# devbib/veles

Measured on AMD Instinct MI355X. Metric: samples/sec (whole node) AlexNet-ImageNet training at 1/2/4/8 MI355X, higher is better.
Workload: dtype bf16; 1 GPU; model=alexnet, global_batch=3072, per_gpu_batch=3072, parallelism=dp1, image=227x227x3, grad_allreduce=none (one rank: no collectives)

## Files before the change

csrc/kernels/wgrad_halo.hip:

```cpp
#include "conv_geom.h"

#ifndef HVK_HALO_ABL
#define HVK_HALO_ABL 0
#endif
#include "fp8_common.h"

using namespace hvk;

namespace {

typedef __attribute__((address_space(3))) s16x4 lds_s16x4;

struct HaloGeom {
  int N, H, W, C, OH, OW, OC, Cg, OCg, KH, KW, pt, pl;
  int P;
  int OHW;
  int KK;
  int Wp;
  int WR;
  int SEGP;
  int spi;
  FastDiv fOW, fWp;
};

template <int MT>
__device__ __forceinline__ int a_sw(int r) {
  if constexpr (MT == 128) return r & 7;
  else if constexpr (MT == 96) return (r >> 2) & 1;
  else return (r >> 1) & 3;
}

typedef __attribute__((address_space(3))) uint8_t lds_u8;

__device__ __forceinline__ bf16x8 tr_read(lds_u8* sm, uint32_t o0,
                                          uint32_t o1) {
  s16x4 lo = __builtin_amdgcn_ds_read_tr16_b64_v4i16((lds_s16x4*)(sm + o0));
  s16x4 hi = __builtin_amdgcn_ds_read_tr16_b64_v4i16((lds_s16x4*)(sm + o1));
  typedef __attribute__((ext_vector_type(8))) short s16x8;
  s16x8 v = __builtin_shufflevector(lo, hi, 0, 1, 2, 3, 4, 5, 6, 7);
  return __builtin_bit_cast(bf16x8, v);
}

template <int MT, int NP, int KHT, int KW, int NJW, int PB, bool SEG,
          bool LEAN>
__global__ void __launch_bounds__(256, 2)
wgrad_halo_kernel(const uint16_t* __restrict__ x,
                  const uint16_t* __restrict__ dy, float* __restrict__ ws,
                  float* __restrict__ wsb, HaloGeom g, int mtiles,
                  int cchunks, int kgroups, int tiles, int kspan,
                  int bias) {
  constexpr int NJ = KHT * KW * NP;
  static_assert(2 * NJW >= NJ, "two wave columns cover the n-tiles");
  constexpr int MI = MT / 32;
  constexpr int AP = MT * 2;
  constexpr int ABYTES = 64 * AP;
  constexpr int NA = ABYTES / 1024;
  static_assert(NA % 4 == 0, "A pieces divide over the four waves");
  constexpr int NAW = NA / 4;
  constexpr int BBYTES = NP * PB;
  constexpr int NB = (BBYTES + 1023) / 1024;
  constexpr int NBW = (NB + 3) / 4;
  constexpr int STAGE = ABYTES + NB * 1024;
  static_assert(2 * 2 * STAGE <= 160 * 1024, "two workgroups per CU");
  __shared__ __attribute__((aligned(16))) uint8_t smem[2 * STAGE];

  const int wgid = xcd_remap(blockIdx.x, gridDim.x);
  const int tile = wgid % tiles;
  const int split = wgid / tiles;
  int tt = tile;
  const int kg = tt % kgroups; tt /= kgroups;
  const int cc = tt % cchunks; tt /= cchunks;
  const int mt = tt % mtiles;
  const int gi = tt / mtiles;
  const int total = SEG ? g.N * g.spi : g.P;
  const int pbeg = split * kspan;
  const int pend = min(total, pbeg + kspan);
  if (pbeg >= pend) return;
  const int coff_y = gi * g.OCg + mt * MT;
  const int coff_x = gi * g.Cg + cc * 16 * NP;
  const int kh0 = kg * KHT;

  const int t = threadIdx.x, lane = t & 63;
  const int w = __builtin_amdgcn_readfirstlane(t >> 6);
  const int wr = w >> 1, wc = w & 1;
  const int fr = lane & 15, fq = lane >> 4;
  const int trq = fr >> 2, trp = fr & 3;
  const int q = fq * 4 + trq;

  lds_u8* sm = (lds_u8*)smem;
  const __amdgpu_buffer_rsrc_t ra = dma_rsrc(dy);
  const __amdgpu_buffer_rsrc_t rb = dma_rsrc(x);

  uint32_t a_off[NAW];
  int a_row[NAW];
#pragma unroll
  for (int i = 0; i < NAW; ++i) {
    const int ib = (w * NAW + i) * 1024 + 16 * lane;
    const int r = ib / AP;
    const int pc = (ib - r * AP) >> 4;
    const int lb = (pc >> 1) ^ a_sw<MT>(r);
    const int m = lb * 16 + (pc & 1) * 8;
    a_row[i] = r;
    a_off[i] = (uint32_t)(r * g.OC + coff_y + m) * 2u;
  }
  const int WS = SEG ? KHT * g.SEGP : g.WR * g.Wp;
  int b_rs[NBW];
  uint32_t b_col[NBW];
  uint32_t b_ok[NBW];
  int b_j[NBW];
#pragma unroll
  for (int i = 0; i < NBW; ++i) {
    const int pi = w + 4 * i;
    const int ib = pi * 1024 + 16 * lane;
    const int plane = ib / PB;
    const int wb = ib - plane * PB;
    const int slot = wb >> 5;
    const int half = (wb >> 4) & 1;
// ... 66 lines not shown
          const uint32_t sj = (uint32_t)(ow + b_j[i]);
          const uint32_t rr = fdiv(sj, g.fWp);
          const int col = (int)(sj - rr * (uint32_t)g.Wp);
          const int ih = ihb + (int)rr + b_rs[i];
          const int iw = col - g.pl;
          const bool ok = b_ok[i] && col < g.OW + g.KW - 1 &&
                          (unsigned)iw < (unsigned)g.W &&
                          (unsigned)ih < (unsigned)g.H;
          const uint32_t v = ok ? (nrow + (uint32_t)ih) * rowbytes +
                                      (uint32_t)iw * pixbytes + b_col[i]
                                : kBufOOB;
          dma16(rb, st + ABYTES + (w + 4 * i) * 1024, v);
        }
      }
      return;
    }
    const int rc = g.OH - oh + KHT - 1;
    const int ih_a = oh + kh0 - g.pt;
    const int ih_b = kh0 - g.pt - rc;
    const int gr_a = n * g.H + ih_a;
    const int gr_b = (n + 1) * g.H + ih_b;
    const bool n1ok = n + 1 < g.N;
#pragma unroll
    for (int i = 0; i < NBW; ++i) {
      if (w + 4 * i < NB) {
        const int rs = b_rs[i];
        const bool first = rs < rc;
        const int ih = (first ? ih_a : ih_b) + rs;
        const int gr = (first ? gr_a : gr_b) + rs;
        const bool ok = b_ok[i] && (unsigned)ih < (unsigned)g.H &&
                        (first || n1ok);
        const uint32_t v = ok ? (uint32_t)gr * rowbytes + b_col[i] : kBufOOB;
        dma16(rb, st + ABYTES + (w + 4 * i) * 1024, v);
      }
    }
  };
  auto advance = [&](uint32_t& n, uint32_t& pin, uint32_t& oh,
                     uint32_t& ow) {
    pin += 64;
    if (SEG && pin >= (uint32_t)g.OHW) {
      pin = 0; oh = 0; ow = 0; ++n;
      return;
    }
    if (!SEG && pin >= (uint32_t)g.OHW) pin -= g.OHW;
    ow += 64;
    while (ow >= (uint32_t)g.OW) {
      ow -= g.OW;
      if (++oh == (uint32_t)g.OH) { oh = 0; ++n; }
    }
  };

  constexpr int kNoRow = 0x40000000;
  int l_rs[NBW], l_bj[NBW];
  uint32_t l_inv[NBW];
  int l_b[4];
  uint32_t l_k[4];
  const uint32_t wp32 = (uint32_t)g.Wp * 32u;
  if constexpr (LEAN) {
#pragma unroll
    for (int i = 0; i < NBW; ++i) {
      if constexpr (SEG) {
        const uint32_t aj = fdiv((uint32_t)b_j[i], g.fWp);
        const int bj = b_j[i] - (int)aj * g.Wp;
        const int r = b_rs[i] + (int)aj;
        l_bj[i] = bj;
        l_rs[i] = b_ok[i] ? r : kNoRow;
        l_inv[i] = (uint32_t)r * rowbytes + (uint32_t)(bj - g.pl) * pixbytes +
                   b_col[i];
      } else {
        l_bj[i] = 0;
        l_rs[i] = b_ok[i] ? b_rs[i] : kNoRow;
        l_inv[i] = (uint32_t)b_rs[i] * rowbytes + b_col[i];
      }
    }
#pragma unroll
    for (int i = 0; i < 4; ++i) {
      const uint32_t c = (uint32_t)(q + 16 * i);
      const uint32_t a = fdiv(c, g.fOW);
      const uint32_t b = c - a * (uint32_t)g.OW;
      l_b[i] = (int)b;
      l_k[i] = (a * (uint32_t)g.Wp + b) * 32u + (uint32_t)(trp * 8 + ABYTES);
    }
  }
  struct LeanStep {
    uint32_t n, pin, oh, ow, base, pa;
    int plim;
  };
  const uint32_t q64 = fdiv(64u, g.fOW), r64 = 64u - q64 * (uint32_t)g.OW;
  const uint32_t inc64 = q64 * rowbytes + (SEG ? r64 * pixbytes : 0u);
  const uint32_t inc_row = rowbytes - (SEG ? (uint32_t)g.OW * pixbytes : 0u);
  const uint32_t inc_img = (uint32_t)(g.H - g.OH) * rowbytes;
  const uint32_t astep = 64u * (uint32_t)g.OC * 2u;
  const uint32_t b_delta = (uint32_t)(g.H - g.OH - KHT + 1) * rowbytes;
  const int b_lo = max(0, g.pt - kh0);
  const int b_len = max(0, g.H + g.pt - kh0 - b_lo);
  const int nb_live = (NB - w + 3) >> 2;
  auto lean_first = [&]() {
    LeanStep s;
    s.n = n0; s.pin = pin0; s.oh = oh0; s.ow = ow0;
    s.base = (n0 * (uint32_t)g.H + oh0 + (uint32_t)(kh0 - g.pt)) * rowbytes +
             (SEG ? ow0 * pixbytes : 0u);
    const uint32_t p = n0 * (uint32_t)g.OHW + pin0;
    s.pa = p * (uint32_t)g.OC * 2u;
    s.plim = SEG ? g.OHW - (int)pin0 : pend - (int)p;
    return s;
  };
  auto lean_issue = [&](const LeanStep& s, uint8_t* st) {
    if constexpr ((HVK_HALO_ABL & 1) != 0) return;
    if (s.plim >= 64) {
#pragma unroll
      for (int i = 0; i < NAW; ++i)
        dma16(ra, st + (w * NAW + i) * 1024, s.pa + a_off[i]);
    } else {
#pragma unroll
      for (int i = 0; i < NAW; ++i) {
        const uint32_t v = (a_row[i] < s.plim) ? s.pa + a_off[i] : kBufOOB;
        dma16(ra, st + (w * NAW + i) * 1024, v);
      }
    }
    if constexpr (SEG) {
      const int ihb = (int)s.oh + kh0 - g.pt;
      const uint32_t cw = (uint32_t)max(0, min(g.W, g.OW + g.KW - 1 - g.pl));
      const uint32_t wrapb = rowbytes - (uint32_t)g.Wp * pixbytes;
#pragma unroll
      for (int i = 0; i < NBW; ++i) {
        bool live = true;
        if (i == NBW - 1 && NB % 4 != 0) {
          int nb = nb_live;
          asm volatile("" : "+s"(nb));
          live = i < nb;
        }
        if (live) {
          const int t = l_bj[i] + (int)s.ow;
          const bool c = t >= g.Wp;
          const uint32_t iw = (uint32_t)(t - (c ? g.Wp + g.pl : g.pl));
          const uint32_t ih = (uint32_t)(l_rs[i] + ihb + (c ? 1 : 0));
          uint32_t a = l_inv[i] + s.base + (c ? wrapb : 0u);
          asm("" : "+v"(a));
          const bool ok = (iw < cw) & (ih < (uint32_t)g.H);
          const uint32_t v = ok ? a : kBufOOB;
          dma16(rb, st + ABYTES + (w + 4 * i) * 1024, v);
        }
      }
      return;
    }
    const int rc = g.OH - (int)s.oh + KHT - 1;
    const int ih_a = (int)s.oh + kh0 - g.pt;
    const int a_lo = max(0, -ih_a);
    const uint32_t a_len = (uint32_t)max(0, min(rc, g.H - ih_a) - a_lo);
    const int bl = rc + b_lo;
    const uint32_t bn = s.n + 1 < (uint32_t)g.N ? (uint32_t)b_len : 0u;
    const uint32_t base_b = s.base + b_delta;
#pragma unroll
    for (int i = 0; i < NBW; ++i) {
      bool live = true;
      if (i == NBW - 1 && NB % 4 != 0) {
        int nb = nb_live;
        asm volatile("" : "+s"(nb));
        live = i < nb;
      }
      if (live) {
        const int rs = l_rs[i];
        uint32_t v = (uint32_t)(rs - bl) < bn ? l_inv[i] + base_b : kBufOOB;
        v = (uint32_t)(rs - a_lo) < a_len ? l_inv[i] + s.base : v;
        dma16(rb, st + ABYTES + (w + 4 * i) * 1024, v);
      }
    }
  };
  auto lean_advance = [&](LeanStep& s) {
    if constexpr (SEG) {
      s.pin += 64;
      if (s.pin >= (uint32_t)g.OHW) {
        s.pa += (uint32_t)s.plim * (uint32_t)g.OC * 2u;
        s.pin = 0; s.oh = 0; s.ow = 0; ++s.n;
        s.base = (s.n * (uint32_t)g.H + (uint32_t)(kh0 - g.pt)) * rowbytes;
        s.plim = g.OHW;
        return;
      }
    } else {
      s.pin += 64;
      if (s.pin >= (uint32_t)g.OHW) s.pin -= g.OHW;
    }
    s.pa += astep;
    s.plim -= 64;
    s.oh += q64;
    s.ow += r64;
    s.base += inc64;
    if (s.ow >= (uint32_t)g.OW) {
      s.ow -= g.OW; ++s.oh; s.base += inc_row;
    }
    if (!SEG && s.oh >= (uint32_t)g.OH) {
      s.oh -= g.OH; ++s.n; s.base += inc_img;
    }
  };

  const int nk = SEG ? pend - pbeg : (pend - pbeg + 63) >> 6;
  LeanStep lc{}, ln{};
  if constexpr (LEAN) {
    lc = lean_first();
    lean_issue(lc, smem);
  } else {
    issue(n0, pin0, oh0, ow0, smem);
  }
  asm volatile("s_waitcnt vmcnt(0)" ::: "memory");
  __builtin_amdgcn_s_barrier();
  asm volatile("" ::: "memory");

  uint32_t nn = n0, pinn = pin0, ohn = oh0, own = ow0;
  if constexpr (LEAN) {
    ln = lc;
    lean_advance(ln);
  } else {
    advance(nn, pinn, ohn, own);
  }

  const bool bwave = bias && kg == 0 && cc == 0 && wc == 0;

  auto main_loop = [&](auto wcc, auto with_bias) {
    constexpr int WC = decltype(wcc)::value;
    constexpr bool WB = decltype(with_bias)::value;
    for (int kt = 0; kt < nk; ++kt) {
      const uint32_t cur = (kt & 1) * STAGE;
      if (kt + 1 < nk) {
        if constexpr (LEAN) lean_issue(ln, smem + ((kt + 1) & 1) * STAGE);
        else issue(nn, pinn, ohn, own, smem + ((kt + 1) & 1) * STAGE);
      }
      uint32_t bb[4][KHT];
      const int kp = SEG ? g.SEGP : g.Wp;
      if constexpr (LEAN) {
        const int thr = g.OW - (int)lc.ow;
        const uint32_t dwp = (uint32_t)(g.Wp - g.OW) * 32u;
        const uint32_t sb = cur + lc.ow * 32u;
        const uint32_t wrap = cur + ABYTES + (uint32_t)(g.OH - (int)lc.oh) * wp32;
#pragma unroll
        for (int i = 0; i < 4; ++i) {
          uint32_t base = l_k[i] + (l_b[i] >= thr ? dwp : 0u);
          if constexpr (SEG) {
            base = q < lc.plim - 16 * i ? base : (uint32_t)(trp * 8 + ABYTES);
            base += cur;
          } else {
            base += sb;
            base += base >= wrap ? (uint32_t)(KHT - 1) * wp32 : 0u;
          }
#pragma unroll
          for (int kh = 0; kh < KHT; ++kh) bb[i][kh] = base + kh * kp * 32;
        }
      } else {
#pragma unroll
      for (int i = 0; i < 4; ++i) {
        const uint32_t ow = ow0 + q + 16 * i;
        const uint32_t gr = fdiv(ow, g.fOW);
        const int owr = (int)(ow - gr * (uint32_t)g.OW);
        int slot;
        if constexpr (SEG) {
          slot = pin0 + q + 16 * i < (uint32_t)g.OHW
                     ? (int)gr * g.Wp + owr - (int)ow0 : 0;
        } else {
          slot = ((int)gr + ((oh0 + gr >= (uint32_t)g.OH) ? KHT - 1 : 0)) *
                     g.Wp + owr;
        }
        const uint32_t base = cur + ABYTES + slot * 32 + trp * 8;
#pragma unroll
        for (int kh = 0; kh < KHT; ++kh) bb[i][kh] = base + kh * kp * 32;
      }
      }
#pragma unroll
      for (int ks = 0; ks < 2; ++ks) {
        bf16x8 a[MI];
#pragma unroll
        for (int i = 0; i < MI; ++i) {
          const uint32_t oa = cur + a_frag[i] + ks * 32 * AP;
          a[i] = tr_read(sm, oa, oa + 16 * AP);
        }
#pragma unroll
        for (int j = 0; j < NJW; ++j) {
          const int jg = WC * NJW + j;
          if (jg < NJ) {
            const int tl = jg / NP, pl_ = jg - (jg / NP) * NP;
            const int khl = tl / KW, kwl = tl - (tl / KW) * KW;
            const uint32_t off = kwl * 32 + pl_ * PB;
            const bf16x8 b = tr_read(sm, bb[2 * ks][khl] + off,
                                     bb[2 * ks + 1][khl] + off);
            if constexpr ((HVK_HALO_ABL & 4) != 0) {
              acc[0][j][0] += (float)b[0] + (float)a[0][0];
            } else {
#pragma unroll
              for (int i = 0; i < MI; ++i)
                acc[i][j] = __builtin_amdgcn_mfma_f32_16x16x32_bf16(
                    b, a[i], acc[i][j], 0, 0, 0);
            }
          }
        }
        if constexpr (WB) {
#pragma unroll
          for (int i = 0; i < MI; ++i)
            accb[i] = __builtin_amdgcn_mfma_f32_16x16x32_bf16(ones, a[i],
                                                              accb[i], 0, 0, 0);
        }
      }
      asm volatile("s_waitcnt vmcnt(0)" ::: "memory");
      __builtin_amdgcn_s_barrier();
      asm volatile("" ::: "memory");
      if constexpr (LEAN) {
        lc = ln;
        lean_advance(ln);
      } else {
        ow0 = own; oh0 = ohn; n0 = nn; pin0 = pinn;
        advance(nn, pinn, ohn, own);
      }
    }
  };
  if (wc == 0) {
    if (bwave) main_loop(std::integral_constant<int, 0>{}, std::true_type{});
    else main_loop(std::integral_constant<int, 0>{}, std::false_type{});
  } else {
    main_loop(std::integral_constant<int, 1>{}, std::false_type{});
  }

  const long long sbase = (long long)split * g.OC;
#pragma unroll
  for (int j = 0; j < NJW; ++j) {
    const int jg = wc * NJW + j;
    if (jg >= NJ || ((HVK_HALO_ABL & 2) && acc[0][j][0] != 1234.5f)) continue;
    const int tl = jg / NP, pl_ = jg - (jg / NP) * NP;
    const int khg = kh0 + tl / KW, kwl = tl - (tl / KW) * KW;
    const int ng = (khg * g.KW + kwl) * g.Cg + cc * 16 * NP + pl_ * 16 + fq * 4;
#pragma unroll
    for (int i = 0; i < MI; ++i) {
      const int mg = coff_y + mrow0 + i * 16 + fr;
      *(float4*)(ws + (sbase + mg) * g.KK + ng) =
          make_float4(acc[i][j][0], acc[i][j][1], acc[i][j][2], acc[i][j][3]);
    }
  }
  if (bwave && fq == 0) {
#pragma unroll
    for (int i = 0; i < MI; ++i)
      wsb[sbase + coff_y + mrow0 + i * 16 + fr] = accb[i][0];
  }
}

template <int R>
__global__ void __launch_bounds__(256)
wgrad_finish_kernel(const float* __restrict__ ws, float* __restrict__ dw,
                    long long n4, int splits, const float* __restrict__ wsb,
                    float* __restrict__ db, int oc, int nmain) {
  constexpr int EPB = 256 / R;
  __shared__ float4 red[256];
  const int r = threadIdx.x % R, el = threadIdx.x / R;
  if ((int)blockIdx.x < nmain) {
    const long long e = (long long)blockIdx.x * EPB + el;
    float4 sacc = make_float4(0.f, 0.f, 0.f, 0.f);
    if (e < n4)
      for (int k = r; k < splits; k += R) {
        const float4 v = ((const float4*)ws)[(long long)k * n4 + e];
        sacc.x += v.x; sacc.y += v.y; sacc.z += v.z; sacc.w += v.w;
      }
    if constexpr (R == 1) {
      if (e < n4) {
        float4 d = ((float4*)dw)[e];
        d.x += sacc.x; d.y += sacc.y; d.z += sacc.z; d.w += sacc.w;
        ((float4*)dw)[e] = d;
      }
      return;
    }
    red[threadIdx.x] = sacc;
    __syncthreads();
    if (r == 0 && e < n4) {
      float4 t = red[el * R];
#pragma unroll
      for (int i = 1; i < R; ++i) {
        const float4 v = red[el * R + i];
        t.x += v.x; t.y += v.y; t.z += v.z; t.w += v.w;
      }
      float4 d = ((float4*)dw)[e];
      d.x += t.x; d.y += t.y; d.z += t.z; d.w += t.w;
      ((float4*)dw)[e] = d;
    }
    return;
  }
  if (db == nullptr) return;
  const int m = ((int)blockIdx.x - nmain) * EPB + el;
  float sb = 0.f;
  if (m < oc)
    for (int k = r; k < splits; k += R) sb += wsb[(long long)k * oc + m];
  float* rf = (float*)red;
  rf[threadIdx.x] = sb;
  __syncthreads();
  if (r == 0 && m < oc) {
    float t = rf[el * R];
    for (int i = 1; i < R; ++i) t += rf[el * R + i];
// ... 276 lines not shown
          accb[i] = __builtin_amdgcn_mfma_scale_f32_16x16x128_f8f6f4(
              ones, a[i], accb[i], FX, FDY, 0, 127, 0, 127);
      }
      asm volatile("s_waitcnt vmcnt(0)" ::: "memory");
      __builtin_amdgcn_s_barrier();
      asm volatile("" ::: "memory");
      ow0 = own; oh0 = ohn; n0 = nn; pin0 = pinn;
      advance(nn, pinn, ohn, own);
    }
  };
  if (wc == 0) {
    if (bwave) main_loop(std::integral_constant<int, 0>{}, std::true_type{});
    else main_loop(std::integral_constant<int, 0>{}, std::false_type{});
  } else {
    main_loop(std::integral_constant<int, 1>{}, std::false_type{});
  }

  const float sdv = fp8_scale(sdys, hist, fmax_dy);
  const float alpha = 1.f / (sdv * fp8_scale(sxs, hist, fmax_x));
  const long long sbase = (long long)split * g.OC;
#pragma unroll
  for (int jn = 0; jn < NJW; ++jn) {
    const int jg = wc * NJW + jn;
    if (jg >= NJ) continue;
    const int tl = jg / NP, pl_ = jg - (jg / NP) * NP;
    const int khg = kh0 + tl / KW, kwl = tl - (tl / KW) * KW;
    const int ng = (khg * g.KW + kwl) * g.Cg + cc * 16 * NP + pl_ * 16 + fg * 4;
#pragma unroll
    for (int i = 0; i < MI; ++i) {
      const int mg = coff_y + mrow0 + i * 16 + fr;
      *(float4*)(ws + (sbase + mg) * g.KK + ng) =
          make_float4(acc[i][jn][0] * alpha, acc[i][jn][1] * alpha,
                      acc[i][jn][2] * alpha, acc[i][jn][3] * alpha);
    }
  }
  if (bwave && fg == 0) {
#pragma unroll
    for (int i = 0; i < MI; ++i)
      wsb[sbase + coff_y + mrow0 + i * 16 + fr] = accb[i][0] / sdv;
  }
}

struct Plan {
  int var;
  int MT, NP, KHT, PB;
  int tiles, mtiles, cchunks, kgroups;
  int splits, kspan;
  HaloGeom g;
};

constexpr int kSlots = 512;
int g_halo_pad = 2;
int g_halo_lean = 1;

Plan make_plan(int N, int H, int W, int C, int OC, int KH, int KW, int pt,
               int pl, int OH, int OW, int groups, int splits,
               bool fp8 = false) {
  const int STEP = fp8 ? 128 : 64, SLOT = fp8 ? 16 : 32, ES = fp8 ? 1 : 2;
  Plan p{};
  const int Cg = C / groups, OCg = OC / groups;
  HaloGeom& g = p.g;
  g.N = N; g.H = H; g.W = W; g.C = C; g.OH = OH; g.OW = OW; g.OC = OC;
  g.Cg = Cg; g.OCg = OCg; g.KH = KH; g.KW = KW; g.pt = pt; g.pl = pl;
  g.P = N * OH * OW;
  g.KK = KH * KW * Cg;
  g.Wp = OW + (fp8 ? 16 : std::max(g_halo_pad, KW - 1));
  g.fOW = make_fastdiv(OW);
  if (OH * OW < STEP || KW > 9 || C % 16 != 0 || OC % 16 != 0) return p;
  if ((long long)N * H * W * C * ES >= kBufMaxBytes ||
      (long long)g.P * OC * ES >= kBufMaxBytes)
    return p;
  g.OHW = OH * OW;
  g.fWp = make_fastdiv(g.Wp);
  const int span = (OW - 1 + STEP - 1) / OW + 1;
  const int cross = (OH * OW) % STEP != 0 ? 2 : 1;
  const int spi = (g.OHW + STEP - 1) / STEP;
  int dmax = 0;
  for (int st = 0; st < spi; ++st) {
    const int pin = STEP * st, last = min(pin + STEP - 1, g.OHW - 1);
    const int d = (last / OW - pin / OW) * g.Wp + last % OW - pin % OW;
    dmax = max(dmax, d);
  }
  struct Cand { int var, MT, NP, KHT, KW, PB, seg; };
  const Cand cands16[] = {
      {1, 128, 2, 3, 3, 7168, 0},
      {5, 128, 2, 3, 3, 7168, 1},
      {4, 128, 2, 3, 3, 10240, 0},
      {2, 96, 2, 3, 3, 7168, 0},
      {7, 96, 3, 3, 3, 8192, 1},
      {6, 64, 4, 3, 3, 7168, 1},
      {3, 128, 3, 1, 5, 5120, 0},
  };
  const Cand cands8[] = {
      {101, 128, 2, 3, 3, 9216, 0},
      {102, 128, 2, 3, 3, 7168, 1},
      {103, 64, 4, 3, 3, 7168, 1},
  };
  const Cand* cands = fp8 ? cands8 : cands16;
  const int ncand = fp8 ? 3 : 7;
  for (int ci = 0; ci < ncand; ++ci) {
    const Cand& c = cands[ci];
    if (KW != c.KW || KH % c.KHT || OCg % c.MT || Cg % (16 * c.NP)) continue;
    if (c.seg) {
      if (spi * STEP * 100 > g.OHW * 103) continue;
      const int segp = dmax + KW;
      if (c.KHT * segp * SLOT > c.PB) continue;
      g.SEGP = segp;
      g.spi = spi;
      g.WR = 0;
    } else {
      const int WR = span + cross * (c.KHT - 1);
      if (WR * g.Wp * SLOT > c.PB) continue;
      g.WR = WR;
      g.SEGP = 0;
      g.spi = 0;
    }
    p.var = c.var; p.MT = c.MT; p.NP = c.NP; p.KHT = c.KHT; p.PB = c.PB;
    break;
  }
  if (!p.var) return p;
  p.mtiles = OCg / p.MT;
  p.cchunks = Cg / (16 * p.NP);
  p.kgroups = KH / p.KHT;
  p.tiles = groups * p.mtiles * p.cchunks * p.kgroups;
  const bool seg = g.SEGP > 0;
  const int steps = seg ? N * spi : (g.P + STEP - 1) / STEP;
  int s = splits > 0 ? splits : kSlots / p.tiles;
  s = max(1, min(s, steps));
  const int ks = (steps + s - 1) / s;
  p.kspan = seg ? ks : ks * STEP;
  p.splits = (steps + ks - 1) / ks;
  return p;
}

}

static long long finish(float* ws, float* wsb, float* dW, float* dbias, int OC,
                 long long kk, int splits, hipStream_t s);

HVK_API long long hvk_conv_wgrad_halo(const void* X, const void* dY, float* dW,
                                      float* dbias, float* ws, int N, int H,
                                      int W, int C, int OC, int KH, int KW,
                                      int pt, int pl, int OH, int OW,
                                      int groups, int splits, hipStream_t s) {
  Plan p = make_plan(N, H, W, C, OC, KH, KW, pt, pl, OH, OW, groups, splits);
  if (!p.var) return -1;
  const long long kk = (long long)KH * KW * (C / groups);
  const long long need = (long long)p.splits * OC * kk + (long long)p.splits * OC;
  if (ws == nullptr) return need;
  if (((uintptr_t)X & 15) || ((uintptr_t)dY & 15)) return -1;
  float* wsb = ws + (long long)p.splits * OC * kk;
  dim3 grid((unsigned)(p.tiles * p.splits)), blk(256);
  const int bias = dbias != nullptr;
  const uint16_t* x = (const uint16_t*)X;
  const uint16_t* dy = (const uint16_t*)dY;
#define HALO_GO1(MT, NP, KHT, KW, NJW, PB, SEG, LEAN)                          \
  hipLaunchKernelGGL(                                                          \
      (wgrad_halo_kernel<MT, NP, KHT, KW, NJW, PB, SEG, LEAN>), grid, blk, 0,  \
      s, x, dy, ws, wsb, p.g, p.mtiles, p.cchunks, p.kgroups, p.tiles,         \
      p.kspan, bias)
#define HALO_GO(MT, NP, KHT, KW, NJW, PB, SEG)                                 \
  if (g_halo_lean) HALO_GO1(MT, NP, KHT, KW, NJW, PB, SEG, true);              \
  else HALO_GO1(MT, NP, KHT, KW, NJW, PB, SEG, false)
  switch (p.var) {
    case 1: HALO_GO(128, 2, 3, 3, 9, 7168, false); break;
    case 2: HALO_GO(96, 2, 3, 3, 9, 7168, false); break;
    case 3: HALO_GO(128, 3, 1, 5, 8, 5120, false); break;
    case 4: HALO_GO(128, 2, 3, 3, 9, 10240, false); break;
    case 5: HALO_GO(128, 2, 3, 3, 9, 7168, true); break;
    case 6: HALO_GO(64, 4, 3, 3, 18, 7168, true); break;
    case 7: HALO_GO(96, 3, 3, 3, 14, 8192, true); break;
    default: return -1;
  }
#undef HALO_GO
#undef HALO_GO1
  hipError_t e = launch_status(s);
  if (e != hipSuccess) return (long long)e;
  return finish(ws, wsb, dW, dbias, OC, kk, p.splits, s);
}

static long long finish(float* ws, float* wsb, float* dW, float* dbias, int OC,
                 long long kk, int splits, hipStream_t s) {
  const long long n4 = (long long)OC * kk / 4;
  const int R = (splits >= 64 && n4 < (1 << 17)) ? 16
              : (splits >= 16 && n4 < (1 << 19)) ? 4 : 1;
  const int epb = 256 / R;
  const int nmain = (int)((n4 + epb - 1) / epb);
  const int nb = dbias ? (OC + epb - 1) / epb : 0;
  auto fk = R == 16 ? wgrad_finish_kernel<16>
          : R == 4 ? wgrad_finish_kernel<4> : wgrad_finish_kernel<1>;
  hipLaunchKernelGGL(fk, dim3(nmain + nb), dim3(256), 0, s, ws, dW, n4,
                     splits, wsb, dbias, OC, nmain);
  return (long long)launch_status(s);
}

HVK_API void hvk_halo_pitch_pad(int p) { g_halo_pad = p; }

HVK_API void hvk_halo_lean(int on) { g_halo_lean = on; }

HVK_API int hvk_conv_wgrad_halo_splits(int N, int H, int W, int C, int OC,
                                       int KH, int KW, int pt, int pl, int OH,
                                       int OW, int groups, int splits) {
  Plan p = make_plan(N, H, W, C, OC, KH, KW, pt, pl, OH, OW, groups, splits);
  return p.var ? p.splits : -1;
}

HVK_API long long hvk_conv_wgrad_halo_fp8(
    const void* X8, const void* dY8, float* dW, float* dbias, float* ws,
    int N, int H, int W, int C, int OC, int KH, int KW, int pt, int pl,
    int OH, int OW, int groups, int splits, int fx, int fdy, const float* sxs,
    const float* sdys, int hist, float fmax_x, float fmax_dy, hipStream_t s) {
  Plan p = make_plan(N, H, W, C, OC, KH, KW, pt, pl, OH, OW, groups, splits,
                     true);
  if (!p.var || (fx != 0 && fx != 1) || (fdy != 0 && fdy != 1)) return -1;
  const long long kk = (long long)KH * KW * (C / groups);
  const long long need = (long long)p.splits * OC * kk + (long long)p.splits * OC;
  if (ws == nullptr) return need;
  if (((uintptr_t)X8 & 15) || ((uintptr_t)dY8 & 15)) return -1;
  float* wsb = ws + (long long)p.splits * OC * kk;
  dim3 grid((unsigned)(p.tiles * p.splits)), blk(256);
  const int bias = dbias != nullptr;
  const uint8_t* x = (const uint8_t*)X8;
  const uint8_t* dy = (const uint8_t*)dY8;
#define HALO8_GO(MT, NP, KHT, KW, NJW, PB, SEG, FX, FDY)                       \
  hipLaunchKernelGGL(                                                          \
      (wgrad_halo8_kernel<MT, NP, KHT, KW, NJW, PB, SEG, FX, FDY>), grid, blk, \
      0, s, x, dy, ws, wsb, p.g, p.mtiles, p.cchunks, p.kgroups, p.tiles,      \
      p.kspan, bias, sxs, sdys, hist, fmax_x, fmax_dy)
#define HALO8_FMT(MT, NP, KHT, KW, NJW, PB, SEG)                               \
  if (fx == 0 && fdy == 1) HALO8_GO(MT, NP, KHT, KW, NJW, PB, SEG, 0, 1);     \
  else if (fx == 0 && fdy == 0) HALO8_GO(MT, NP, KHT, KW, NJW, PB, SEG, 0, 0); \
  else if (fx == 1 && fdy == 1) HALO8_GO(MT, NP, KHT, KW, NJW, PB, SEG, 1, 1); \
  else HALO8_GO(MT, NP, KHT, KW, NJW, PB, SEG, 1, 0)
  switch (p.var) {
    case 101: HALO8_FMT(128, 2, 3, 3, 9, 9216, false); break;
    case 102: HALO8_FMT(128, 2, 3, 3, 9, 7168, true); break;
    case 103: HALO8_FMT(64, 4, 3, 3, 18, 7168, true); break;
    default: return -1;
  }
#undef HALO8_FMT
#undef HALO8_GO
  hipError_t e = launch_status(s);
  if (e != hipSuccess) return (long long)e;
  return finish(ws, wsb, dW, dbias, OC, kk, p.splits, s);
}
```

veles_amd/ops/__init__.py:

```python
from __future__ import annotations

import math
import os
import struct

import torch
import torch.nn.functional as F

from veles_amd.ops import _lib
from veles_amd.ops._lib import available, require_library

__all__ = ["ACT", "gemm", "linear_fwd", "conv_out_size", "conv_fwd",
           "conv_dgrad", "conv_wgrad", "col_sum", "row_sum", "act_fwd",
           "act_bwd", "pool_fwd", "pool_bwd", "lrn_fwd", "lrn_bwd",
           "softmax_ce", "mse", "sgd_update", "dropout", "xorshift1024star",
           "xorshift128plus", "join", "cast", "fill_minibatch",
           "mean_disp_normalize", "act_code", "kohonen_coords",
           "kohonen_argmin", "kohonen_update", "lstm_fwd", "lstm_bwd",
           "rbm_layout", "rbm_uniforms", "rbm_sample", "rbm_grad",
           "bn_partials", "batchnorm_fwd", "batchnorm_bwd", "attention_fwd",
           "attention_bwd", "mha_fwd", "mha_bwd", "attn_head_dim"]

DT = {torch.float32: 0, torch.bfloat16: 1, torch.uint8: 2, torch.int32: 3,
      torch.float16: 4}
# ... 999 lines not shown
        if isinstance(col, (S2DImage, PaddedImage)):
            col = None
        if col is not None:
            K = KH * KW * Cg
            M = N * OH * OW
            sp = splits or wgrad_splits(M, OC, K, 1)
            gemm(dy.reshape(M, OC), col[:, :K], trans_a=True,
                 out=dw.view(OC, K), accumulate=True, splits=sp,
                 bias_grad=dbias)
            return dw
        if needs_im2col(C, groups):
            runp = (KW * C + 7) // 8 * 8
            sp = splits or _wgrad_splits_for(
                x, dy, dw, sliding, padding, groups,
                (N * OH * OW, OC, KH * runp + 1, 1))
            _lib_call("hvk_conv_wgrad_run", _p(x), _p(dy), _p(dw), _p(dbias),
                      N, H, W, C, OC, KH, KW, sy, sx, pt, pl, OH, OW,
                      int(sp), _s(x))
            return dw
        if (sy, sx) == (1, 1) and _halo_wgrad(x, dy, dw, dbias, N, H, W, C,
                                               OC, KH, KW, pt, pl, OH, OW,
                                               groups, splits):
            return dw
        if splits is None:
            splits = _wgrad_splits_for(
                x, dy, dw, sliding, padding, groups,
                (N * OH * OW, OC // groups, KH * KW * Cg + 1, groups))
        _lib_call("hvk_conv_wgrad", _p(x), _p(dy), _p(dw), N, H, W, C, OC, KH,
                  KW, sy, sx, pt, pl, OH, OW, groups, int(splits), _p(dbias),
                  _s(x))
        return dw
    xp = F.pad(_nchw(x), (pl, pr, pt, pb))
    g = torch.nn.grad.conv2d_weight(xp, (OC, Cg, KH, KW), _nchw(dy),
                                    stride=(sy, sx), groups=groups)
    dw += g.permute(0, 2, 3, 1)
    if dbias is not None:
        dbias += dy.float().reshape(-1, OC).sum(0)
    return dw


_HALO_WGRAD = os.environ.get("VELES_AMD_HALO_WGRAD", "1") != "0"


def set_halo_wgrad(on):
    global _HALO_WGRAD
    _HALO_WGRAD = bool(on)


def set_halo_wgrad_lean(on):
    if _lib.available():
        _lib.lib().hvk_halo_lean(int(bool(on)))


def _halo_wgrad(x, dy, dw, dbias, N, H, W, C, OC, KH, KW, pt, pl, OH, OW,
                groups, splits=None):
    if not _HALO_WGRAD or x.dtype != torch.bfloat16 or \
            dy.dtype != torch.bfloat16 or not dw.is_contiguous() or \
            not x.is_contiguous() or not dy.is_contiguous() or \
            x.data_ptr() % 16 or dy.data_ptr() % 16:
        return False
    from veles_amd.ops import _lib
    fn = _lib.lib().hvk_conv_wgrad_halo
    geo = (N, H, W, C, OC, KH, KW, pt, pl, OH, OW, groups,
           int(splits) if splits else 0)
    need = fn(_p(x), _p(dy), _p(dw), _p(dbias), None, *geo, _s(x))
    if need < 0:
        return False
    ws = _grow_ws("wgrad_halo_ws", int(need), torch.float32, x.device)
    rc = fn(_p(x), _p(dy), _p(dw), _p(dbias), _p(ws), *geo, _s(x))
    _lib.check(int(rc), "hvk_conv_wgrad_halo")
    return True


_WGRAD_BLOCKS = int(os.environ.get("HVK_WGRAD_BLOCKS", "512"))


def _wgrad_splits_for(x, dy, dw, sliding, padding, groups, shape):
    from veles_amd.ops import autotune
    default = wgrad_splits(*shape)
    autotune.log_call("wgrad", shape, {
        "x": tuple(x if isinstance(x, tuple) else x.shape), "dy": tuple(dy.shape), "dw": tuple(dw.shape),
        "sliding": tuple(sliding), "padding": tuple(padding),
        "groups": groups, "default": default})
    t = autotune.lookup("wgrad", *shape)
    if deterministic():
        return 1
    return default if t is None else max(1, t)


def wgrad_splits(P, M, N, groups, target_blocks=None):
    if deterministic():
        return 1
    target_blocks = target_blocks or _WGRAD_BLOCKS
    tiles = ((M + 127) // 128) * ((N + 127) // 128) * groups
    splits = max(1, min(target_blocks // max(tiles, 1), P // 256))
    return splits


def col_sum(x2d, out=None, scale=1.0, accumulate=False):
    R, C = x2d.shape
    if out is None:
        out = torch.zeros(C, dtype=torch.float32, device=x2d.device)
    elif not accumulate:
        out.zero_()
    if _gpu(x2d) and not deterministic():
        _lib_call("hvk_col_sum", _p(x2d), DT[x2d.dtype], R, C, _p(out),
# ... 2501 lines not shown
```

veles_amd/ops/_lib.py:

```python
from __future__ import annotations

import ctypes
import os
import threading

from veles_amd.error import KernelLibraryMissing

_HERE = os.path.dirname(os.path.abspath(__file__))
LIB_PATH = os.environ.get("HVK_LIBRARY", os.path.join(_HERE, "libhvk.so"))

_lib = None
_lock = threading.Lock()

P = ctypes.c_void_p
I = ctypes.c_int
L = ctypes.c_longlong
F = ctypes.c_float
D = ctypes.c_double
U = ctypes.c_uint

_SIGS = {
    "hvk_gemm": [I, I, I, I, I, P, I, P, I, P, I, I, I, F, F, P, I, I, P, I, I,
                 I, P, P],
    "hvk_gemm_splitk": [I, I, I, I, I, P, I, P, I, P, I, I, F, P, I, P, I, I,
# ... 39 lines not shown
    "hvk_space_to_depth": [P, P] + [I] * 9 + [P],
    "hvk_s2d_weights": [P, P] + [I] * 5 + [P],
    "hvk_s2d_grad_fold": [P, P] + [I] * 6 + [P],
    "hvk_pool_fwd": [P, P, P] + [I] * 13 + [P],
    "hvk_pool_bwd": [P, P, P] + [I] * 13 + [P, I, P],
    "hvk_lrn_fwd": [P, P, L, I, I, F, F, F, P],
    "hvk_lrn_bwd": [P, P, P, L, I, I, F, F, F, P, I, P],
    "hvk_lrn_pool_fwd": [P, P, P] + [I] * 9 + [F, F, F, P],
    "hvk_lrn_pool_bwd": [P, P, P, P] + [I] * 9 + [F, F, F, P, I, P],
    "hvk_pool2_fwd": [P, P] + [I] * 5 + [P],
    "hvk_pool2_fwd_q8": [P, P] + [I] * 5 + [P, P, P, F, I, I, P],
    "hvk_stochastic_pool": [P, P, P] + [I] * 12 + [P, P],
    "hvk_pool2_bwd": [P, P, P] + [I] * 5 + [P, I, P],
    "hvk_pool2_bwd_q8": [P, P, P] + [I] * 5 + [P, I, P, P, P, F, I, I, P],
    "hvk_lrn_pool_fwd_u8": [P, P, P] + [I] * 7 + [F, F, F, P],
    "hvk_lrn_pool_bwd_u8": [P, P, P, P] + [I] * 7 + [F, F, F, P, I, P],
    "hvk_gemm_f32": [I, I, I, I, I, P, I, P, I, P, I, F, F, I, P],
    "hvk_gemm_f64": [I, I, I, I, I, P, I, P, I, P, I, D, D, I, P],
    "hvk_fp8_quant": [P, I, L, P, I, P, I, F, I, P],
    "hvk_fp8_amax": [P, I, L, P, I, P],
    "hvk_fp8_roll": [P, I, I, I, I, P, P],
    "hvk_fp8_roll_dev": [P, I, I, P, P, P],
    "hvk_gemm_fp8": [I, I, I, P, I, I, P, I, I, P, I, P, I, P, I, I, P, P, I,
                     F, F, P],
    "hvk_conv_fwd_fp8": [P, P, P, P] + [I] * 17 + [P, P, I, F, F,
                                                  P, P, P, F, I, P],
    "hvk_conv_dgrad_fp8": [P, P, P] + [I] * 14 + [P, I, I, I, P, P, I, F, F,
                           P, P, P, F, I, P],
    "hvk_conv_wgrad_fp8": [P, P, P, P] + [I] * 17 + [P, P, I, F, F, P],
    "hvk_conv_wgrad_halo": [P, P, P, P, P] + [I] * 13 + [P],
    "hvk_conv_wgrad_halo_splits": [I] * 13,
    "hvk_conv_wgrad_halo_fp8": [P, P, P, P, P] + [I] * 15 + [P, P, I, F, F,
                                                            P],
    "hvk_conv_fwd_hc": [P, P, P, P] + [I] * 13 + [P, P],
    "hvk_conv_dgrad_hc": [P, P, P] + [I] * 12 + [P, I, P, P],
    "hvk_conv_dgrad_hc_w": [P, P, P] + [I] * 12 + [P, I, P, P],
    "hvk_conv_hc_wpack_bytes": [I] * 14,
    "hvk_hc_variant": [I],
    "hvk_hc_pitch_pad": [I],
    "hvk_hc32": [I],
    "hvk_halo_pitch_pad": [I],
    "hvk_hc32_ts": [I],
    "hvk_transpose_colsum": [P, I, I, P, P, I, P, P],
    "hvk_hc_last_variant": [],
    "hvk_set_pool_bwd_variant": [I],
    "hvk_hc_ablation": [I],
    "hvk_take_last_error": [],
    "hvk_end_stream_capture": [P],
    "hvk_stream_create": [],
}
_OPTIONAL = {
    "hvk_hc32_handover": [I],
    "hvk_halo_lean": [I],
    "hvk_hc_max_wgs": [I],
    "hvk_hc_stamps": [P],
    "hvk_kohonen_argmin": [P, I, P, I, I, I, I, P, P, P, P, I, P],
    "hvk_kohonen_update": [P, I, P, P, P, I, I, I, I, F, F, P, I, P],
    "hvk_lstm_step_fwd": [I, I, I] + [P, L] * 7 + [P],
    "hvk_lstm_step_bwd": [I, I, I] + [P, L] * 9 + [P],
    "hvk_recurrent_fn": [I, P, P, L, P],
    "hvk_gru_step_fwd": [I, I] + [P, L] * 8 + [P, P],
    "hvk_gru_step_bwd": [I, I] + [P, L] * 10 + [P],
    "hvk_lstm_step_fwd2": [I, I, I] + [P, L] * 14 + [P],
    "hvk_lstm_step_bwd2": [I, I, I] + [P, L] * 18 + [P],
    "hvk_gru_step_fwd2": [I, I] + ([P, L] * 8 + [P]) * 2 + [P],
    "hvk_gru_step_bwd2": [I, I] + [P, L] * 20 + [P],
    "hvk_rbm_sample": [I, I, I, I, P, L, P, L, P, P, L, P, L, U, P, L, P],
    "hvk_rbm_grad_splits": [I, I, I, I],
    "hvk_rbm_grad": [I, I, I] + [P, L] * 4 + [P, F, P, I, P],
    "hvk_solver4": [P, P, P, P, P, P, I, L, F, L, P, F, P],
    "hvk_grad_sqnorm": [P, L, P, I, P, P],
    "hvk_bn_partials": [L, I, I],
    "hvk_bn_vec": [P, L, I],
    "hvk_bn_stats": [P, L, L, I, I, P, P, P, P, F, F, P, P, P, P, P],
    "hvk_bn_fold": [P, P, P, P, I, F, P, P],
    "hvk_bn_apply": [P, L, P, L, L, I, P, I, P],
    "hvk_bn_bwd": [P, L] * 5 + [L, I, I, P, P, P, P, P, I, I, I, P, P, P],
    "hvk_attn_tile": [I],
    "hvk_attn_fwd": [P, L] * 4 + [P, I, I, I, I, I, P],
    "hvk_attn_bwd_delta": [P, L] * 2 + [P, I, I, I, I, P],
    "hvk_attn_bwd_dkv": [P, L] * 4 + [P, P] + [P, L] * 2 + [I, I, I, I, I, P],
    "hvk_attn_bwd_dq": [P, L] * 4 + [P, P] + [P, L] + [I, I, I, I, I, P],
}
_PTR_RET = {"hvk_stream_create"}
_LL_RET = {"hvk_conv_wgrad_halo", "hvk_conv_wgrad_halo_fp8",
           "hvk_conv_hc_wpack_bytes"}


def _load():
    global _lib
    with _lock:
        if _lib is not None:
            return _lib
        if not os.path.exists(LIB_PATH):
            return None
        lib = ctypes.CDLL(LIB_PATH)
        for name, sig in _SIGS.items():
            fn = getattr(lib, name, None)
            if fn is None:
                raise KernelLibraryMissing("%s lacks %s - rebuild with python "
                                           "-m veles_amd.ops.build" %
                                           (LIB_PATH, name))
            fn.argtypes = sig
            fn.restype = ctypes.c_void_p if name in _PTR_RET else \
                ctypes.c_longlong if name in _LL_RET else ctypes.c_int
        for name, sig in _OPTIONAL.items():
# ... 52 lines not shown
```

Baseline: 207,600 samples/s.

## Split halo wgrad double buffer into two LDS objects with unrolled even/odd steps

Adds an STG variant of the lean halo weight-gradient kernel. The two pipeline stages become separate LDS arrays and the main loop is unrolled into even/odd steps, so each step uses a constant buffer base instead of computing a per-iteration offset. It also switches to a typed LDS buffer-load DMA, packs row and column indices into one register to cut VGPR use, reads both k-slices of A fragments up front, and uses a precise waitcnt encoding. It is enabled by default for variants 1, 2 and 7. The cost is more code and register pressure from holding both A slices, plus a risk of changing how waits interleave with MFMA work.

```diff
diff --git a/csrc/kernels/wgrad_halo.hip b/csrc/kernels/wgrad_halo.hip
--- a/csrc/kernels/wgrad_halo.hip
+++ b/csrc/kernels/wgrad_halo.hip
@@ -32,6 +32,12 @@
 
 typedef __attribute__((address_space(3))) uint8_t lds_u8;
 
+__device__ __forceinline__ void dma16l(__amdgpu_buffer_rsrc_t r, lds_u8* lds,
+                                       uint32_t voff) {
+  __builtin_amdgcn_raw_ptr_buffer_load_lds(
+      r, (__attribute__((address_space(3))) void*)lds, 16, voff, 0, 0, 0);
+}
+
 __device__ __forceinline__ bf16x8 tr_read(lds_u8* sm, uint32_t o0,
                                           uint32_t o1) {
   s16x4 lo = __builtin_amdgcn_ds_read_tr16_b64_v4i16((lds_s16x4*)(sm + o0));
@@ -42,7 +48,7 @@
 }
 
 template <int MT, int NP, int KHT, int KW, int NJW, int PB, bool SEG,
-          bool LEAN>
+          bool LEAN, bool STG>
 __global__ void __launch_bounds__(256, 2)
 wgrad_halo_kernel(const uint16_t* __restrict__ x,
                   const uint16_t* __restrict__ dy, float* __restrict__ ws,
@@ -62,7 +68,11 @@
   constexpr int NBW = (NB + 3) / 4;
   constexpr int STAGE = ABYTES + NB * 1024;
   static_assert(2 * 2 * STAGE <= 160 * 1024, "two workgroups per CU");
-  __shared__ __attribute__((aligned(16))) uint8_t smem[2 * STAGE];
+  static_assert(LEAN || !STG, "the two-object stages are the lean loop's");
+  static_assert(STAGE % 1024 == 0, "whole DMA pieces per stage");
+  __shared__ __attribute__((aligned(1024))) uint8_t
+      smem[STG ? STAGE : 2 * STAGE];
+  __shared__ __attribute__((aligned(1024))) uint8_t smem1[STG ? STAGE : 16];
 
   const int wgid = xcd_remap(blockIdx.x, gridDim.x);
   const int tile = wgid % tiles;
@@ -235,6 +245,7 @@
 
   constexpr int kNoRow = 0x40000000;
   int l_rs[NBW], l_bj[NBW];
+  uint32_t l_pk[NBW];
   uint32_t l_inv[NBW];
   int l_b[4];
   uint32_t l_k[4];
@@ -248,10 +259,12 @@
         const int r = b_rs[i] + (int)aj;
         l_bj[i] = bj;
         l_rs[i] = b_ok[i] ? r : kNoRow;
+        l_pk[i] = b_ok[i] ? (uint32_t)bj | (uint32_t)r << 16 : 0xffffffffu;
         l_inv[i] = (uint32_t)r * rowbytes + (uint32_t)(bj - g.pl) * pixbytes +
                    b_col[i];
       } else {
         l_bj[i] = 0;
+        l_pk[i] = 0;
         l_rs[i] = b_ok[i] ? b_rs[i] : kNoRow;
         l_inv[i] = (uint32_t)b_rs[i] * rowbytes + b_col[i];
       }
@@ -263,6 +276,10 @@
       const uint32_t b = c - a * (uint32_t)g.OW;
       l_b[i] = (int)b;
       l_k[i] = (a * (uint32_t)g.Wp + b) * 32u + (uint32_t)(trp * 8 + ABYTES);
+      if constexpr (STG) {
+        l_k[i] |= b << 16;
+        asm volatile("" : "+v"(l_k[i]));
+      }
     }
   }
   struct LeanStep {
@@ -288,17 +305,20 @@
     s.plim = SEG ? g.OHW - (int)pin0 : pend - (int)p;
     return s;
   };
-  auto lean_issue = [&](const LeanStep& s, uint8_t* st) {
+  auto lean_issue = [&](const LeanStep& s, lds_u8* st) {
     if constexpr ((HVK_HALO_ABL & 1) != 0) return;
     if (s.plim >= 64) {
 #pragma unroll
       for (int i = 0; i < NAW; ++i)
-        dma16(ra, st + (w * NAW + i) * 1024, s.pa + a_off[i]);
+        dma16l(ra, st + (w * NAW + i) * 1024, s.pa + a_off[i]);
     } else {
+      int la = lane;
+      if constexpr (STG) asm volatile("" : "+v"(la));
 #pragma unroll
       for (int i = 0; i < NAW; ++i) {
-        const uint32_t v = (a_row[i] < s.plim) ? s.pa + a_off[i] : kBufOOB;
-        dma16(ra, st + (w * NAW + i) * 1024, v);
+        const int r = STG ? ((w * NAW + i) * 1024 + 16 * la) / AP : a_row[i];
+        const uint32_t v = (r < s.plim) ? s.pa + a_off[i] : kBufOOB;
+        dma16l(ra, st + (w * NAW + i) * 1024, v);
       }
     }
     if constexpr (SEG) {
@@ -314,15 +334,17 @@
           live = i < nb;
         }
         if (live) {
-          const int t = l_bj[i] + (int)s.ow;
+          const int bj = STG ? (int)(l_pk[i] & 0xffffu) : l_bj[i];
+          const int rs = STG ? (int)(l_pk[i] >> 16) : l_rs[i];
+          const int t = bj + (int)s.ow;
           const bool c = t >= g.Wp;
           const uint32_t iw = (uint32_t)(t - (c ? g.Wp + g.pl : g.pl));
-          const uint32_t ih = (uint32_t)(l_rs[i] + ihb + (c ? 1 : 0));
+          const uint32_t ih = (uint32_t)(rs + ihb + (c ? 1 : 0));
           uint32_t a = l_inv[i] + s.base + (c ? wrapb : 0u);
           asm("" : "+v"(a));
           const bool ok = (iw < cw) & (ih < (uint32_t)g.H);
           const uint32_t v = ok ? a : kBufOOB;
-          dma16(rb, st + ABYTES + (w + 4 * i) * 1024, v);
+          dma16l(rb, st + ABYTES + (w + 4 * i) * 1024, v);
         }
       }
       return;
@@ -346,7 +368,7 @@
         const int rs = l_rs[i];
         uint32_t v = (uint32_t)(rs - bl) < bn ? l_inv[i] + base_b : kBufOOB;
         v = (uint32_t)(rs - a_lo) < a_len ? l_inv[i] + s.base : v;
-        dma16(rb, st + ABYTES + (w + 4 * i) * 1024, v);
+        dma16l(rb, st + ABYTES + (w + 4 * i) * 1024, v);
       }
     }
   };
@@ -377,15 +399,24 @@
     }
   };
 
+  auto stage_wait = [&]() {
+    if constexpr (STG) {
+      asm volatile("" ::: "memory");
+      __builtin_amdgcn_s_waitcnt(0x0f70);
+      asm volatile("" ::: "memory");
+    } else {
+      asm volatile("s_waitcnt vmcnt(0)" ::: "memory");
+    }
+  };
   const int nk = SEG ? pend - pbeg : (pend - pbeg + 63) >> 6;
   LeanStep lc{}, ln{};
   if constexpr (LEAN) {
     lc = lean_first();
-    lean_issue(lc, smem);
+    lean_issue(lc, sm);
   } else {
     issue(n0, pin0, oh0, ow0, smem);
   }
-  asm volatile("s_waitcnt vmcnt(0)" ::: "memory");
+  stage_wait();
   __builtin_amdgcn_s_barrier();
   asm volatile("" ::: "memory");
 
@@ -397,16 +428,28 @@
     advance(nn, pinn, ohn, own);
   }
 
-  const bool bwave = bias && kg == 0 && cc == 0 && wc == 0;
+  constexpr int BWC = STG ? 1 : 0;
+  const bool bwave = bias && kg == 0 && cc == 0 && wc == BWC;
 
   auto main_loop = [&](auto wcc, auto with_bias) {
     constexpr int WC = decltype(wcc)::value;
     constexpr bool WB = decltype(with_bias)::value;
-    for (int kt = 0; kt < nk; ++kt) {
-      const uint32_t cur = (kt & 1) * STAGE;
-      if (kt + 1 < nk) {
-        if constexpr (LEAN) lean_issue(ln, smem + ((kt + 1) & 1) * STAGE);
-        else issue(nn, pinn, ohn, own, smem + ((kt + 1) & 1) * STAGE);
+    auto step = [&](auto par, int kt, bool more) {
+      constexpr int PAR = decltype(par)::value;
+      const uint32_t cur = STG ? 0 : (kt & 1) * STAGE;
+      lds_u8* sc;
+      if constexpr (!STG) sc = sm;
+      else if constexpr (PAR == 0) sc = (lds_u8*)smem;
+      else sc = (lds_u8*)smem1;
+      if (more) {
+        if constexpr (STG) {
+          if constexpr (PAR == 0) lean_issue(ln, (lds_u8*)smem1);
+          else lean_issue(ln, (lds_u8*)smem);
+        } else if constexpr (LEAN) {
+          lean_issue(ln, sm + ((kt + 1) & 1) * STAGE);
+        } else {
+          issue(nn, pinn, ohn, own, smem + ((kt + 1) & 1) * STAGE);
+        }
       }
       uint32_t bb[4][KHT];
       const int kp = SEG ? g.SEGP : g.Wp;
@@ -417,7 +460,12 @@
         const uint32_t wrap = cur + ABYTES + (uint32_t)(g.OH - (int)lc.oh) * wp32;
 #pragma unroll
         for (int i = 0; i < 4; ++i) {
-          uint32_t base = l_k[i] + (l_b[i] >= thr ? dwp : 0u);
+          uint32_t base;
+          if constexpr (STG)
+            base = (l_k[i] & 0xffffu) +
+                   (l_k[i] >= (uint32_t)thr << 16 ? dwp : 0u);
+          else
+            base = l_k[i] + (l_b[i] >= thr ? dwp : 0u);
           if constexpr (SEG) {
             base = q < lc.plim - 16 * i ? base : (uint32_t)(trp * 8 + ABYTES);
             base += cur;
@@ -447,14 +495,15 @@
         for (int kh = 0; kh < KHT; ++kh) bb[i][kh] = base + kh * kp * 32;
       }
       }
-#pragma unroll
-      for (int ks = 0; ks < 2; ++ks) {
-        bf16x8 a[MI];
-#pragma unroll
-        for (int i = 0; i < MI; ++i) {
-          const uint32_t oa = cur + a_frag[i] + ks * 32 * AP;
-          a[i] = tr_read(sm, oa, oa + 16 * AP);
-        }
+      if constexpr (STG) {
+        bf16x8 a[2][MI];
+#pragma unroll
+        for (int ks = 0; ks < 2; ++ks)
+#pragma unroll
+          for (int i = 0; i < MI; ++i) {
+            const uint32_t oa = a_frag[i] + ks * 32 * AP;
+            a[ks][i] = tr_read(sc, oa, oa + 16 * AP);
+          }
 #pragma unroll
         for (int j = 0; j < NJW; ++j) {
           const int jg = WC * NJW + j;
@@ -462,7 +511,46 @@
             const int tl = jg / NP, pl_ = jg - (jg / NP) * NP;
             const int khl = tl / KW, kwl = tl - (tl / KW) * KW;
             const uint32_t off = kwl * 32 + pl_ * PB;
-            const bf16x8 b = tr_read(sm, bb[2 * ks][khl] + off,
+#pragma unroll
+            for (int ks = 0; ks < 2; ++ks) {
+              const bf16x8 b = tr_read(sc, bb[2 * ks][khl] + off,
+                                       bb[2 * ks + 1][khl] + off);
+              if constexpr ((HVK_HALO_ABL & 4) != 0) {
+                acc[0][j][0] += (float)b[0] + (float)a[ks][0][0];
+              } else {
+#pragma unroll
+                for (int i = 0; i < MI; ++i)
+                  acc[i][j] = __builtin_amdgcn_mfma_f32_16x16x32_bf16(
+                      b, a[ks][i], acc[i][j], 0, 0, 0);
+              }
+            }
+          }
+        }
+        if constexpr (WB) {
+#pragma unroll
+          for (int ks = 0; ks < 2; ++ks)
+#pragma unroll
+            for (int i = 0; i < MI; ++i)
+              accb[i] = __builtin_amdgcn_mfma_f32_16x16x32_bf16(
+                  ones, a[ks][i], accb[i], 0, 0, 0);
+        }
+      } else {
+#pragma unroll
+      for (int ks = 0; ks < 2; ++ks) {
+        bf16x8 a[MI];
+#pragma unroll
+        for (int i = 0; i < MI; ++i) {
+          const uint32_t oa = cur + a_frag[i] + ks * 32 * AP;
+          a[i] = tr_read(sc, oa, oa + 16 * AP);
+        }
+#pragma unroll
+        for (int j = 0; j < NJW; ++j) {
+          const int jg = WC * NJW + j;
+          if (jg < NJ) {
+            const int tl = jg / NP, pl_ = jg - (jg / NP) * NP;
+            const int khl = tl / KW, kwl = tl - (tl / KW) * KW;
+            const uint32_t off = kwl * 32 + pl_ * PB;
+            const bf16x8 b = tr_read(sc, bb[2 * ks][khl] + off,
                                      bb[2 * ks + 1][khl] + off);
             if constexpr ((HVK_HALO_ABL & 4) != 0) {
               acc[0][j][0] += (float)b[0] + (float)a[0][0];
@@ -481,25 +569,44 @@
                                                               accb[i], 0, 0, 0);
         }
       }
-      asm volatile("s_waitcnt vmcnt(0)" ::: "memory");
+      }
+      stage_wait();
       __builtin_amdgcn_s_barrier();
       asm volatile("" ::: "memory");
       if constexpr (LEAN) {
         lc = ln;
         lean_advance(ln);
+        if constexpr (STG)
+          asm volatile("" : "+s"(ln.n), "+s"(ln.pin), "+s"(ln.oh), "+s"(ln.ow),
+                            "+s"(ln.base), "+s"(ln.pa), "+s"(ln.plim));
       } else {
         ow0 = own; oh0 = ohn; n0 = nn; pin0 = pinn;
         advance(nn, pinn, ohn, own);
       }
+    };
+    constexpr std::integral_constant<int, 0> even{};
+    constexpr std::integral_constant<int, 1> odd{};
+    if constexpr (STG) {
+      int kt = 0;
+      for (; kt + 1 < nk; kt += 2) {
+        step(even, kt, true);
+        step(odd, kt + 1, kt + 2 < nk);
+      }
+      if (kt < nk) step(even, kt, false);
+    } else {
+      for (int kt = 0; kt < nk; ++kt) step(even, kt, kt + 1 < nk);
     }
   };
-  if (wc == 0) {
-    if (bwave) main_loop(std::integral_constant<int, 0>{}, std::true_type{});
-    else main_loop(std::integral_constant<int, 0>{}, std::false_type{});
+  if (wc == BWC) {
+    if (bwave) main_loop(std::integral_constant<int, BWC>{}, std::true_type{});
+    else main_loop(std::integral_constant<int, BWC>{}, std::false_type{});
   } else {
-    main_loop(std::integral_constant<int, 1>{}, std::false_type{});
-  }
-
+    main_loop(std::integral_constant<int, 1 - BWC>{}, std::false_type{});
+  }
+
+  int te = threadIdx.x;
+  if constexpr (STG) asm volatile("" : "+v"(te));
+  const int fre = STG ? te & 15 : fr, fqe = STG ? (te & 63) >> 4 : fq;
   const long long sbase = (long long)split * g.OC;
 #pragma unroll
   for (int j = 0; j < NJW; ++j) {
@@ -507,18 +614,18 @@
     if (jg >= NJ || ((HVK_HALO_ABL & 2) && acc[0][j][0] != 1234.5f)) continue;
     const int tl = jg / NP, pl_ = jg - (jg / NP) * NP;
     const int khg = kh0 + tl / KW, kwl = tl - (tl / KW) * KW;
-    const int ng = (khg * g.KW + kwl) * g.Cg + cc * 16 * NP + pl_ * 16 + fq * 4;
+    const int ng = (khg * g.KW + kwl) * g.Cg + cc * 16 * NP + pl_ * 16 + fqe * 4;
 #pragma unroll
     for (int i = 0; i < MI; ++i) {
-      const int mg = coff_y + mrow0 + i * 16 + fr;
+      const int mg = coff_y + mrow0 + i * 16 + fre;
       *(float4*)(ws + (sbase + mg) * g.KK + ng) =
           make_float4(acc[i][j][0], acc[i][j][1], acc[i][j][2], acc[i][j][3]);
     }
   }
-  if (bwave && fq == 0) {
+  if (bwave && fqe == 0) {
 #pragma unroll
     for (int i = 0; i < MI; ++i)
-      wsb[sbase + coff_y + mrow0 + i * 16 + fr] = accb[i][0];
+      wsb[sbase + coff_y + mrow0 + i * 16 + fre] = accb[i][0];
   }
 }
 
@@ -901,6 +1008,7 @@
 constexpr int kSlots = 512;
 int g_halo_pad = 2;
 int g_halo_lean = 1;
+int g_halo_stages = 1;
 
 Plan make_plan(int N, int H, int W, int C, int OC, int KH, int KW, int pt,
                int pl, int OH, int OW, int groups, int splits,
@@ -1003,24 +1111,30 @@
   const int bias = dbias != nullptr;
   const uint16_t* x = (const uint16_t*)X;
   const uint16_t* dy = (const uint16_t*)dY;
-#define HALO_GO1(MT, NP, KHT, KW, NJW, PB, SEG, LEAN)                          \
+#define HALO_GO1(MT, NP, KHT, KW, NJW, PB, SEG, LEAN, STG)                     \
   hipLaunchKernelGGL(                                                          \
-      (wgrad_halo_kernel<MT, NP, KHT, KW, NJW, PB, SEG, LEAN>), grid, blk, 0,  \
-      s, x, dy, ws, wsb, p.g, p.mtiles, p.cchunks, p.kgroups, p.tiles,         \
-      p.kspan, bias)
+      (wgrad_halo_kernel<MT, NP, KHT, KW, NJW, PB, SEG, LEAN, STG>), grid,     \
+      blk, 0, s, x, dy, ws, wsb, p.g, p.mtiles, p.cchunks, p.kgroups,          \
+      p.tiles, p.kspan, bias)
 #define HALO_GO(MT, NP, KHT, KW, NJW, PB, SEG)                                 \
-  if (g_halo_lean) HALO_GO1(MT, NP, KHT, KW, NJW, PB, SEG, true);              \
-  else HALO_GO1(MT, NP, KHT, KW, NJW, PB, SEG, false)
+  if (g_halo_lean && g_halo_stages)                                            \
+    HALO_GO1(MT, NP, KHT, KW, NJW, PB, SEG, true, true);                       \
+  else if (g_halo_lean) HALO_GO1(MT, NP, KHT, KW, NJW, PB, SEG, true, false);  \
+  else HALO_GO1(MT, NP, KHT, KW, NJW, PB, SEG, false, false)
+#define HALO_GO_ONE(MT, NP, KHT, KW, NJW, PB, SEG)                             \
+  if (g_halo_lean) HALO_GO1(MT, NP, KHT, KW, NJW, PB, SEG, true, false);       \
+  else HALO_GO1(MT, NP, KHT, KW, NJW, PB, SEG, false, false)
   switch (p.var) {
     case 1: HALO_GO(128, 2, 3, 3, 9, 7168, false); break;
     case 2: HALO_GO(96, 2, 3, 3, 9, 7168, false); break;
-    case 3: HALO_GO(128, 3, 1, 5, 8, 5120, false); break;
-    case 4: HALO_GO(128, 2, 3, 3, 9, 10240, false); break;
-    case 5: HALO_GO(128, 2, 3, 3, 9, 7168, true); break;
-    case 6: HALO_GO(64, 4, 3, 3, 18, 7168, true); break;
+    case 3: HALO_GO_ONE(128, 3, 1, 5, 8, 5120, false); break;
+    case 4: HALO_GO_ONE(128, 2, 3, 3, 9, 10240, false); break;
+    case 5: HALO_GO_ONE(128, 2, 3, 3, 9, 7168, true); break;
+    case 6: HALO_GO_ONE(64, 4, 3, 3, 18, 7168, true); break;
     case 7: HALO_GO(96, 3, 3, 3, 14, 8192, true); break;
     default: return -1;
   }
+#undef HALO_GO_ONE
 #undef HALO_GO
 #undef HALO_GO1
   hipError_t e = launch_status(s);
@@ -1046,6 +1160,8 @@
 HVK_API void hvk_halo_pitch_pad(int p) { g_halo_pad = p; }
 
 HVK_API void hvk_halo_lean(int on) { g_halo_lean = on; }
+
+HVK_API void hvk_halo_stages(int on) { g_halo_stages = on; }
 
 HVK_API int hvk_conv_wgrad_halo_splits(int N, int H, int W, int C, int OC,
                                        int KH, int KW, int pt, int pl, int OH,
diff --git a/veles_amd/ops/__init__.py b/veles_amd/ops/__init__.py
--- a/veles_amd/ops/__init__.py
+++ b/veles_amd/ops/__init__.py
@@ -1075,6 +1075,11 @@
         _lib.lib().hvk_halo_lean(int(bool(on)))
 
 
+def set_halo_wgrad_stages(on):
+    if _lib.available():
+        _lib.lib().hvk_halo_stages(int(bool(on)))
+
+
 def _halo_wgrad(x, dy, dw, dbias, N, H, W, C, OC, KH, KW, pt, pl, OH, OW,
                 groups, splits=None):
     if not _HALO_WGRAD or x.dtype != torch.bfloat16 or \
diff --git a/veles_amd/ops/_lib.py b/veles_amd/ops/_lib.py
--- a/veles_amd/ops/_lib.py
+++ b/veles_amd/ops/_lib.py
@@ -115,6 +115,7 @@
 _OPTIONAL = {
     "hvk_hc32_handover": [I],
     "hvk_halo_lean": [I],
+    "hvk_halo_stages": [I],
     "hvk_hc_max_wgs": [I],
     "hvk_hc_stamps": [P],
     "hvk_kohonen_argmin": [P, I, P, I, I, I, I, P, P, P, P, I, P],
```

New measurement: 210,800 samples/s (median of 6 runs). +1.6%, better.
